# JohnVinyard/music-synthesis

Measured on AMD Instinct MI355X. Metric: GAN train-step audio samples/sec (22.05 kHz, 8192-sample window), higher is better.
Workload: dtype f32 storage and accumulate; multiplies on the 16-bit matrix pipe with split fp32 operands: block-scaled fp16 x 2 (22 significand bits, 3 products per multiply) in the atoms, the k5 layer, the grouped convs, the stride-8 transposed forward and the atom weight gradients; exact bf16 x 3 (6 products) or; 1 GPU; stage-2 GAN train step: alternating D/G trainer calls, MelGAN generator + 3-scale discriminator + feature-matching loss (BASELINE.json configs[2]); per_gpu_batch=32, global_batch=32, window=8192, mels=80, optimizer=FlatAdam(1e-4,(0.5,0.9)), parallelism=dp1, hipgraph=True

## Files before the change

### music-synthesis_amd/csrc/conv5_img.hip

```cpp
#include "operand_split.h"
#include <stdlib.h>

namespace {

constexpr int K5 = 5;
constexpr int PX_MAX = 350;
constexpr int R_MAX = 64;
constexpr int W_NPART = 256;
__host__ __device__ inline size_t c5_tail_u4(int M, int CK) { return (size_t)(M / 32) * (CK / 16) * 5 * 2 * 64; }

__global__ __launch_bounds__(256) void k_conv5_wmax(const float* __restrict__ W, size_t n, float* __restrict__ pm) {
    __shared__ float red[4];
    const size_t per = (n + W_NPART - 1) / W_NPART, lo = blockIdx.x * per, hi = lo + per < n ? lo + per : n;
    float m = 0.f;
    size_t i = lo + 4 * (size_t)threadIdx.x;
    for (; i + 3 < hi; i += 1024) {
        const f32x4u v = *reinterpret_cast<const f32x4u*>(W + i);
        m = fmaxf(fmaxf(m, fmaxf(fabsf(v[0]), fabsf(v[1]))), fmaxf(fabsf(v[2]), fabsf(v[3])));
    }
    for (; i < hi; ++i) m = fmaxf(m, fabsf(W[i]));
#pragma unroll
    for (int o = 32; o > 0; o >>= 1) m = fmaxf(m, __shfl_xor(m, o, 64));
    if ((threadIdx.x & 63) == 0) red[threadIdx.x >> 6] = m;
    __syncthreads();
    if (threadIdx.x == 0) pm[blockIdx.x] = fmaxf(fmaxf(red[0], red[1]), fmaxf(red[2], red[3]));
}

__global__ __launch_bounds__(256) void k_conv5_pack(const float* __restrict__ W, u32x4* __restrict__ img, int M, int CK,
                                                   int backward, int np, const float* __restrict__ pm) {
    const int NC = CK / 16;
    const size_t idx = (size_t)blockIdx.x * 256 + threadIdx.x;
    const size_t total = (size_t)(M / 32) * NC * K5 * 64;
    float WS = 1.f, iWS = 1.f;
    if (np == 2) {
        float* tail = reinterpret_cast<float*>(img + c5_tail_u4(M, CK));
        weight_scale(weight_max256(pm ? pm : tail), WS, iWS);
        if (idx == 0) tail[W_NPART] = iWS;
    }
    if (idx >= total) return;
    const int lane = (int)(idx & 63);
    size_t r = idx >> 6;
    const int tap = (int)(r % K5); r /= K5;
    const int chunk = (int)(r % NC);
    const int ms = (int)(r / NC);
    const int row = ms * 32 + (lane & 31), k0 = chunk * 16 + 8 * (lane >> 5);
    unsigned pc[3][4];
#pragma unroll
    for (int q = 0; q < 4; ++q) {
        float a, b;
        if (!backward) {
            a = W[((size_t)row * CK + k0 + 2 * q) * K5 + tap];
            b = W[((size_t)row * CK + k0 + 2 * q + 1) * K5 + tap];
        } else {
            a = W[((size_t)(k0 + 2 * q) * M + row) * K5 + (K5 - 1 - tap)];
            b = W[((size_t)(k0 + 2 * q + 1) * M + row) * K5 + (K5 - 1 - tap)];
        }
        if (np == 3) {
            unsigned o[3];
            split_pair<3>(a, b, o);
            pc[0][q] = o[0]; pc[1][q] = o[1]; pc[2][q] = o[2];
        } else {
            unsigned o[2];
            split_pair<2>(a * WS, b * WS, o);
            pc[0][q] = o[0]; pc[1][q] = o[1]; pc[2][q] = 0u;
        }
    }
    u32x4* dst = img + ((size_t)((ms * NC + chunk) * K5 + tap) * np) * 64 + lane;
    for (int pp = 0; pp < np; ++pp) dst[pp * 64] = u32x4{pc[pp][0], pc[pp][1], pc[pp][2], pc[pp][3]};
}

struct C5P {
    int B, M, CK, L;
    int R, SS, PX;
    int NV, NVG;
    int cks, nsplit;
    int act;
    float slope;
    long long zstride;
};

extern __shared__ __attribute__((aligned(16))) unsigned char smem5[];

template <int MODE, int NP, bool PRE = false>
__device__ __forceinline__ void conv5_body(const C5P& p, const float* __restrict__ X, const float* __restrict__ Xact,
                                           const u32x4* __restrict__ IMG, const float* __restrict__ bias,
                                           const float* __restrict__ add, float* __restrict__ Y,
                                           float* __restrict__ slabs, int bx, const u32x4* __restrict__ P = nullptr,
                                           const float* __restrict__ Pinv = nullptr) {
    constexpr int XRS = xrs<NP>();
    constexpr bool SC = NP == 2;
    static_assert(!PRE || NP == 2, "pre-split operands are fp16 pieces");
    const int tid = threadIdx.x, lane = tid & 63, h = lane >> 5, l31 = lane & 31;
    const int wid = __builtin_amdgcn_readfirstlane(tid >> 6);
    const int wm = wid >> 2, wn = wid & 3;
    const int L = p.L, b0 = bx * p.R, m0 = blockIdx.y * 64;
    const int cbeg = blockIdx.z * p.cks;
    const int cend = cbeg + p.cks < p.CK ? cbeg + p.cks : p.CK;
    const int nchunks = (cend - cbeg) / 16;
// ... 687 lines not shown
```

### music-synthesis_amd/csrc/conv_thin.hip

```cpp
#include "ms_common.h"
#include "conv_thin.h"
#include <stdlib.h>

namespace {

constexpr int TS = 1024;

template <int K, bool FLIP, bool VEC, int CW>
__global__ __launch_bounds__(256) void k_thin_reduce(int B, int C, int L, int s_kind, int act,
                                                    float slope, const float* __restrict__ S,
                                                    const float* __restrict__ Sact,
                                                    const float* __restrict__ w,
                                                    const float* __restrict__ bias,
                                                    const float* __restrict__ res,
                                                    float* __restrict__ out) {
    constexpr int OFF = (K - 1) / 2;
    constexpr int HV = (OFF + 3) / 4;
    constexpr int NV = 2 * HV + 1;
    constexpr int NW = VEC ? NV * 4 : K + 3;
    constexpr int W0 = VEC ? 4 * HV : OFF;
    __shared__ float red[4][256 + 4];
    const int lane = threadIdx.x & 63, wid = threadIdx.x >> 6;
    const int tiles = (L + 255) / 256;
    const int b = blockIdx.x / tiles, t = (blockIdx.x - b * tiles) * 256 + lane * 4;
// ... 11 lines not shown
                const int tq = t + 4 * (q - HV);
                const bool ok = tq >= 0 && tq < L;
                const float4 v = *reinterpret_cast<const float4*>(S + row + (ok ? tq : 0));
                win[cc][4 * q + 0] = v.x; win[cc][4 * q + 1] = v.y; win[cc][4 * q + 2] = v.z; win[cc][4 * q + 3] = v.w;
            }
        } else {
#pragma unroll
            for (int i = 0; i < K + 3; ++i) {
                const int ti = t + i - OFF;
                const bool ok = ti >= 0 && ti < L;
                win[cc][i] = S[row + (ok ? ti : 0)];
            }
        }
    }
    if (Sact) {
        float wa[CW][NW];
#pragma unroll
        for (int cc = 0; cc < CW; ++cc) {
            const int c = wid * CW + cc;
            const size_t row = ((size_t)b * C + (c < C ? c : 0)) * L;
            if (VEC) {
#pragma unroll
                for (int q = 0; q < NV; ++q) {
                    const int tq = t + 4 * (q - HV);
                    const bool ok = tq >= 0 && tq < L;
                    const float4 v = *reinterpret_cast<const float4*>(Sq + row + (ok ? tq : 0));
                    wa[cc][4 * q + 0] = v.x; wa[cc][4 * q + 1] = v.y; wa[cc][4 * q + 2] = v.z; wa[cc][4 * q + 3] = v.w;
                }
            } else {
#pragma unroll
                for (int i = 0; i < K + 3; ++i) {
                    const int ti = t + i - OFF;
                    const bool ok = ti >= 0 && ti < L;
                    wa[cc][i] = Sq[row + (ok ? ti : 0)];
                }
            }
        }
#pragma unroll
        for (int cc = 0; cc < CW; ++cc)
#pragma unroll
            for (int i = 0; i < NW; ++i) win[cc][i] = ms_act_grad(win[cc][i], wa[cc][i], kind, slope);
    }
#pragma unroll
    for (int cc = 0; cc < CW; ++cc) {
        const int c = wid * CW + cc;
        if (c >= C) continue;
#pragma unroll
        for (int i = 0; i < NW; ++i) {
            const int ti = t + i - W0;
            if (ti < 0 || ti >= L) win[cc][i] = 0.f;
        }
#pragma unroll
        for (int j = 0; j < K; ++j) {
            const float wv = w[c * K + (FLIP ? K - 1 - j : j)];
#pragma unroll
            for (int e = 0; e < 4; ++e) acc[e] = fmaf(wv, win[cc][W0 + e + j - OFF], acc[e]);
        }
    }
#pragma unroll
    for (int e = 0; e < 4; ++e) red[wid][lane * 4 + e] = acc[e];
    __syncthreads();
    const int to = (blockIdx.x - b * tiles) * 256 + threadIdx.x;
    if (to < L) {
        const int i = threadIdx.x;
        float v = (red[0][i] + red[1][i]) + (red[2][i] + red[3][i]);
        v = ms_apply_act(v + (bias ? bias[0] : 0.f), act, slope);
        const size_t o = (size_t)b * L + to;
        if (res) v += res[o];
        out[o] = v;
    }
}

template <int K, bool FLIP, bool VEC, int CW>
__global__ __launch_bounds__(256) void k_thin_expand(int B, int C, int L, int t_kind, int act,
                                                    float slope, const float* __restrict__ T,
                                                    const float* __restrict__ Tact,
                                                    const float* __restrict__ w,
                                                    const float* __restrict__ bias,
                                                    const float* __restrict__ add,
                                                    float* __restrict__ out) {
    constexpr int OFF = (K - 1) / 2;
    const int lane = threadIdx.x & 63, wid = threadIdx.x >> 6;
    const int tiles = (L + 255) / 256;
    const int b = blockIdx.x / tiles, s = (blockIdx.x - b * tiles) * 256 + lane * 4;
    if (s >= L) return;
    const float* Tq = Tact ? Tact : T;
    const int kind = Tact ? t_kind : MS_ACT_NONE;
    float v[K + 3], a[K + 3], win[K + 3];
#pragma unroll
    for (int i = 0; i < K + 3; ++i) {
        const int ti = s + i - OFF;
        const bool ok = ti >= 0 && ti < L;
        v[i] = T[(size_t)b * L + (ok ? ti : 0)];
        a[i] = Tq[(size_t)b * L + (ok ? ti : 0)];
    }
#pragma unroll
    for (int i = 0; i < K + 3; ++i) {
        const int ti = s + i - OFF;
        const bool ok = ti >= 0 && ti < L;
        win[i] = ok ? ms_act_grad(v[i], a[i], kind, slope) : 0.f;
    }
    float4 av[CW];
    if (add && VEC) {
#pragma unroll
        for (int cc = 0; cc < CW; ++cc) {
            const int c = wid * CW + cc;
            av[cc] = *reinterpret_cast<const float4*>(add + ((size_t)b * C + (c < C ? c : 0)) * L + s);
        }
    }
#pragma unroll
    for (int cc = 0; cc < CW; ++cc) {
        const int c = wid * CW + cc;
        if (c >= C) continue;
        float acc[4] = {0.f, 0.f, 0.f, 0.f};
#pragma unroll
        for (int j = 0; j < K; ++j) {
            const float wv = w[c * K + (FLIP ? K - 1 - j : j)];
#pragma unroll
            for (int e = 0; e < 4; ++e) acc[e] = fmaf(wv, win[e + j], acc[e]);
        }
        const float bv = bias ? bias[c] : 0.f;
        const size_t o = ((size_t)b * C + c) * L + s;
        float r[4];
#pragma unroll
        for (int e = 0; e < 4; ++e) r[e] = ms_apply_act(acc[e] + bv, act, slope);
        if (VEC) {
            if (add) { r[0] += av[cc].x; r[1] += av[cc].y; r[2] += av[cc].z; r[3] += av[cc].w; }
            *reinterpret_cast<float4*>(out + o) = make_float4(r[0], r[1], r[2], r[3]);
        } else {
#pragma unroll
            for (int e = 0; e < 4; ++e)
                if (s + e < L) out[o + e] = r[e] + (add ? add[o + e] : 0.f);
        }
    }
}

template <int K, int ROLE, int CPW, bool VEC>
__global__ __launch_bounds__(256) void k_thin_wgrad(int B, int C, int L, int pad, int act, float slope,
                                                   int schunks, const float* __restrict__ S,
                                                   const float* __restrict__ Sact,
                                                   const float* __restrict__ T,
                                                   const float* __restrict__ Tact,
                                                   float* __restrict__ partial, size_t pstride) {
    constexpr int TW = TS + K - 1;
    constexpr int NT = (TW + 255) / 256;
    __shared__ float Tl[NT * 256];
    __shared__ float red[4];
    const int tid = threadIdx.x, lane = tid & 63, wid = tid >> 6;
    const int b = blockIdx.x / schunks, s0 = (blockIdx.x - b * schunks) * TS;
    const int lo = ROLE == 0 ? s0 - (K - 1) + pad : s0 - pad;
    const float* Tq = Tact ? Tact : T;
    const int t_kind = Tact ? act : MS_ACT_NONE;
    const float* Sq = Sact ? Sact : S;
    const int s_kind = Sact ? act : MS_ACT_NONE;
    float bs = 0.f;
    {
        float tv[NT], ta[NT];
#pragma unroll
        for (int it = 0; it < NT; ++it) {
            const int i = tid + it * 256, t = lo + i;
            const bool ok = i < TW && t >= 0 && t < L;
            tv[it] = T[(size_t)b * L + (ok ? t : 0)];
            ta[it] = Tq[(size_t)b * L + (ok ? t : 0)];
        }
#pragma unroll
        for (int it = 0; it < NT; ++it) {
            const int i = tid + it * 256, t = lo + i;
            const bool ok = i < TW && t >= 0 && t < L;
            const float v = ok ? ms_act_grad(tv[it], ta[it], t_kind, slope) : 0.f;
            Tl[i] = v;
            if (ROLE == 0 && ok && t >= s0 && t < s0 + TS) bs += v;
        }
    }
    __syncthreads();
    float acc[CPW][K];
    float bsum[CPW];
#pragma unroll
    for (int cc = 0; cc < CPW; ++cc) {
        bsum[cc] = 0.f;
#pragma unroll
        for (int j = 0; j < K; ++j) acc[cc][j] = 0.f;
    }
    const int c0 = wid * CPW;
#pragma unroll 1
    for (int pass = 0; pass < TS / 256; ++pass) {
        const int sl = pass * 256 + lane * 4, s = s0 + sl;
        float win[K + 3];
#pragma unroll
        for (int i = 0; i < K + 3; ++i) win[i] = Tl[sl + i];
        float4 sv[CPW], sa[CPW];
#pragma unroll
        for (int cc = 0; cc < CPW; ++cc) {
            const int c = c0 + cc;
            const bool ok = c < C && s < L;
            const size_t o = ok ? ((size_t)b * C + c) * L + s : 0;
            if (VEC) {
                sv[cc] = *reinterpret_cast<const float4*>(S + o);
                sa[cc] = *reinterpret_cast<const float4*>(Sq + o);
            } else {
                const size_t o1 = ok && s + 1 < L ? o + 1 : o, o2 = ok && s + 2 < L ? o + 2 : o,
                             o3 = ok && s + 3 < L ? o + 3 : o;
                sv[cc] = make_float4(S[o], S[o1], S[o2], S[o3]);
                sa[cc] = make_float4(Sq[o], Sq[o1], Sq[o2], Sq[o3]);
            }
        }
#pragma unroll
        for (int cc = 0; cc < CPW; ++cc) {
            const int c = c0 + cc;
            const float xv[4] = {sv[cc].x, sv[cc].y, sv[cc].z, sv[cc].w};
            const float xa[4] = {sa[cc].x, sa[cc].y, sa[cc].z, sa[cc].w};
#pragma unroll
            for (int e = 0; e < 4; ++e) {
                const bool ok = c < C && s + e < L;
                const float v = ok ? ms_act_grad(xv[e], xa[e], s_kind, slope) : 0.f;
                bsum[cc] += v;
#pragma unroll
                for (int j = 0; j < K; ++j)
                    acc[cc][j] = fmaf(v, win[ROLE == 0 ? e + K - 1 - j : e + j], acc[cc][j]);
            }
        }
    }
    float* prow = partial + (size_t)blockIdx.x * pstride;
#pragma unroll
    for (int cc = 0; cc < CPW; ++cc) {
        const int c = c0 + cc;
#pragma unroll
        for (int j = 0; j < K; ++j) {
            const float r = ms_wave_sum(acc[cc][j]);
            if (lane == 0 && c < C) prow[c * K + j] = r;
        }
        if (ROLE == 1) {
            const float r = ms_wave_sum(bsum[cc]);
            if (lane == 0 && c < C) prow[(size_t)C * K + c] = r;
        }
    }
    if (ROLE == 0) {
        const float tot = ms_block_sum(bs, red);
        if (tid == 0) prow[(size_t)C * K] = tot;
    }
}

template <int LT>
__global__ __launch_bounds__(256) void k_thin_short_fwd(int C, int L, int act, float slope,
                                                       const float* __restrict__ x,
                                                       const float* __restrict__ w,
                                                       const float* __restrict__ bias,
                                                       float* __restrict__ y) {
    __shared__ float red[4][LT];
    const int tid = threadIdx.x, lane = tid & 63, wid = tid >> 6, b = blockIdx.x;
    float acc[LT];
#pragma unroll
    for (int t = 0; t < LT; ++t) acc[t] = 0.f;
    for (int c = tid; c < C; c += 256) {
        const float w0 = w[c * 3], w1 = w[c * 3 + 1], w2 = w[c * 3 + 2];
        const float* row = x + ((size_t)b * C + c) * L;
        float v[LT + 2];
        v[0] = 0.f;
#pragma unroll
        for (int t = 0; t < LT; ++t) v[t + 1] = t < L ? row[t < L ? t : 0] : 0.f;
        v[LT + 1] = 0.f;
#pragma unroll
        for (int t = 0; t < LT; ++t) acc[t] += w0 * v[t] + w1 * v[t + 1] + w2 * v[t + 2];
    }
#pragma unroll
    for (int t = 0; t < LT; ++t) {
        const float sred = ms_wave_sum(acc[t]);
        if (lane == 0) red[wid][t] = sred;
    }
// ... 331 lines not shown
```

### music-synthesis_amd/csrc/disc_parts.hip

```cpp
#include "operand_split.h"
#include "gconv_mfma.h"
#include <stdint.h>
#include <stdlib.h>

namespace {

constexpr int NP = MS_CONV_PARTS_MAX;

struct DParts {
    int count, wg0[NP + 1];
    int B[NP], L[NP], tiles[NP];
    const float* a[NP];
    const float* b[NP];
    const float* c[NP];
    float* o[NP];
};

struct DPart {
    int B, L, tiles, wg;
    const float* a;
    const float* b;
    const float* c;
    float* o;
};
__device__ __forceinline__ DPart pick_part(const DParts& q, int wg) {
    DPart p{q.B[0], q.L[0], q.tiles[0], wg, q.a[0], q.b[0], q.c[0], q.o[0]};
#pragma unroll
    for (int k = 1; k < NP; ++k)
        if (k < q.count && wg >= q.wg0[k]) p = DPart{q.B[k], q.L[k], q.tiles[k], wg - q.wg0[k], q.a[k], q.b[k], q.c[k], q.o[k]};
    return p;
}

__device__ __forceinline__ float lrelu_grad(float g, float y, float slope) { return y > 0.f ? g : g * slope; }

constexpr int FK = 15, FPAD = 7, FC = 16, FT = 1024;

__device__ __forceinline__ void stage_thin_window(float* xs, const float* x, int B, int L, int b, int tile_t) {
    const auto rs = __builtin_amdgcn_make_buffer_rsrc(const_cast<float*>(x), 0, 4u * (unsigned)(B * L), 0x00020000);
    for (int i = threadIdx.x; i < (FT + 16) / 4; i += 256) {
        const int t = tile_t - 8 + 4 * i;
        *reinterpret_cast<f32x4*>(xs + 4 * i) = load_row4(rs, (unsigned)(b * L), t, L);
    }
    __syncthreads();
}

__global__ __launch_bounds__(256) void k_dfirst_fwd(DParts q, const float* __restrict__ w, const float* __restrict__ bias,
                                                   float slope) {
    __shared__ __attribute__((aligned(16))) float xs[FT + 16];
    const DPart p = pick_part(q, blockIdx.x);
    const int b = p.wg / p.tiles, tile_t = (p.wg - b * p.tiles) * FT;
    stage_thin_window(xs, p.a, p.B, p.L, b, tile_t);
    const int t0 = tile_t + 4 * threadIdx.x;
    if (t0 >= p.L) return;
    float win[20];
#pragma unroll
    for (int i = 0; i < 5; ++i) {
        const f32x4 v = *reinterpret_cast<const f32x4*>(xs + 4 * threadIdx.x + 4 * i);
        win[4 * i] = v[0]; win[4 * i + 1] = v[1]; win[4 * i + 2] = v[2]; win[4 * i + 3] = v[3];
    }
    const bool whole = t0 + 3 < p.L;
#pragma unroll 4
    for (int co = 0; co < FC; ++co) {
        float v[4];
        const float bv = bias ? bias[co] : 0.f;
#pragma unroll
        for (int e = 0; e < 4; ++e) v[e] = bv;
#pragma unroll
        for (int k = 0; k < FK; ++k) {
            const float wk = w[co * FK + k];
#pragma unroll
            for (int e = 0; e < 4; ++e) v[e] = fmaf(wk, win[1 + e + k], v[e]);
        }
#pragma unroll
        for (int e = 0; e < 4; ++e) v[e] = fmaxf(v[e], v[e] * slope);
        float* yr = p.o + ((size_t)b * FC + co) * p.L + t0;
        if (whole) {
            *reinterpret_cast<f32x4u*>(yr) = (f32x4u){v[0], v[1], v[2], v[3]};
        } else {
#pragma unroll
            for (int e = 0; e < 4; ++e)
                if (t0 + e < p.L) yr[e] = v[e];
        }
    }
}

__global__ __launch_bounds__(256) void k_dfirst_bwd_data(DParts q, const float* __restrict__ w, float slope) {
    __shared__ float red[4][256 + 4];
    const DPart p = pick_part(q, blockIdx.x);
    const int lane = threadIdx.x & 63, wid = threadIdx.x >> 6;
    const int b = p.wg / p.tiles, tile_t = (p.wg - b * p.tiles) * 256;
    const int t0 = tile_t + 4 * lane;
    const unsigned bytes = 4u * (unsigned)(p.B * FC * p.L);
    const auto rsG = __builtin_amdgcn_make_buffer_rsrc(const_cast<float*>(p.a), 0, bytes, 0x00020000);
    const auto rsY = __builtin_amdgcn_make_buffer_rsrc(const_cast<float*>(p.b), 0, bytes, 0x00020000);
    float acc[4] = {0.f, 0.f, 0.f, 0.f};
#pragma unroll
    for (int cc = 0; cc < 4; ++cc) {
        const int co = wid * 4 + cc;
        const unsigned row = (unsigned)((b * FC + co) * p.L);
        float win[20];
#pragma unroll
        for (int i = 0; i < 5; ++i) {
            const f32x4 g = load_row4(rsG, row, t0 - 8 + 4 * i, p.L);
            const f32x4 y = load_row4(rsY, row, t0 - 8 + 4 * i, p.L);
#pragma unroll
            for (int e = 0; e < 4; ++e) win[4 * i + e] = lrelu_grad(g[e], y[e], slope);
        }
#pragma unroll
        for (int k = 0; k < FK; ++k) {
            const float wk = w[co * FK + k];
#pragma unroll
            for (int e = 0; e < 4; ++e) acc[e] = fmaf(wk, win[8 + e + FPAD - k], acc[e]);
        }
    }
#pragma unroll
    for (int e = 0; e < 4; ++e) red[wid][4 * lane + e] = acc[e];
    __syncthreads();
    const int to = tile_t + threadIdx.x;
    if (to < p.L) {
        const int i = threadIdx.x;
        float v = (red[0][i] + red[1][i]) + (red[2][i] + red[3][i]);
        if (p.c) v += p.c[(size_t)b * p.L + to];
        p.o[(size_t)b * p.L + to] = v;
    }
}

__global__ __launch_bounds__(256) void k_dfirst_wgrad(DParts q, float slope, float* __restrict__ partial) {
    __shared__ __attribute__((aligned(16))) float xs[FT + 16];
    const int lane = threadIdx.x & 63, wid = threadIdx.x >> 6;
    float acc[4][FK], bsum[4];
#pragma unroll
    for (int cc = 0; cc < 4; ++cc) {
        bsum[cc] = 0.f;
#pragma unroll
        for (int k = 0; k < FK; ++k) acc[cc][k] = 0.f;
    }
    const int nunits = q.wg0[q.count];
    for (int unit = blockIdx.x; unit < nunits; unit += gridDim.x) {
        const DPart p = pick_part(q, unit);
        const int b = p.wg / p.tiles, tile_t = (p.wg - b * p.tiles) * FT;
        __syncthreads();
        stage_thin_window(xs, p.a, p.B, p.L, b, tile_t);
        const unsigned bytes = 4u * (unsigned)(p.B * FC * p.L);
        const auto rsG = __builtin_amdgcn_make_buffer_rsrc(const_cast<float*>(p.b), 0, bytes, 0x00020000);
        const auto rsY = __builtin_amdgcn_make_buffer_rsrc(const_cast<float*>(p.c), 0, bytes, 0x00020000);
#pragma unroll 1
        for (int pass = 0; pass < FT / 256; ++pass) {
            const int sl = pass * 256 + 4 * lane, t0 = tile_t + sl;
            if (tile_t + pass * 256 >= p.L) break;
            float win[20];
#pragma unroll
            for (int i = 0; i < 5; ++i) {
                const f32x4 v = *reinterpret_cast<const f32x4*>(xs + sl + 4 * i);
                win[4 * i] = v[0]; win[4 * i + 1] = v[1]; win[4 * i + 2] = v[2]; win[4 * i + 3] = v[3];
            }
            f32x4 g[4], y[4];
#pragma unroll
            for (int cc = 0; cc < 4; ++cc) {
                const unsigned row = (unsigned)((b * FC + wid * 4 + cc) * p.L);
                g[cc] = load_row4(rsG, row, t0, p.L);
                y[cc] = load_row4(rsY, row, t0, p.L);
            }
#pragma unroll
            for (int cc = 0; cc < 4; ++cc)
#pragma unroll
                for (int e = 0; e < 4; ++e) {
                    const float v = lrelu_grad(g[cc][e], y[cc][e], slope);
                    bsum[cc] += v;
#pragma unroll
                    for (int k = 0; k < FK; ++k) acc[cc][k] = fmaf(v, win[1 + e + k], acc[cc][k]);
                }
        }
    }
    float* prow = partial + (size_t)blockIdx.x * (FC * FK + FC);
#pragma unroll
    for (int cc = 0; cc < 4; ++cc) {
        const int co = wid * 4 + cc;
#pragma unroll
        for (int k = 0; k < FK; ++k) {
            const float r = ms_wave_sum(acc[cc][k]);
            if (lane == 0) prow[co * FK + k] = r;
        }
        const float r = ms_wave_sum(bsum[cc]);
        if (lane == 0) prow[FC * FK + co] = r;
    }
}

__global__ __launch_bounds__(256) void k_dparts_reduce(const float* __restrict__ partial, int nslabs, int stride, int nw,
                                                      int nb, float* __restrict__ gw, float* __restrict__ gb, float beta) {
    const int lane = threadIdx.x & 63, i = blockIdx.x * 4 + (threadIdx.x >> 6);
    if (i >= nw + nb) return;
    float s = 0.f;
    for (int z = lane; z < nslabs; z += 64) s += partial[(size_t)z * stride + i];
    s = ms_wave_sum(s);
    if (lane == 0 && (i < nw || gb)) {
        float* dst = i < nw ? gw + i : gb + (i - nw);
        *dst = (beta != 0.f ? beta * *dst : 0.f) + s;
    }
}

constexpr int JL = 32, JP = 33;

__device__ __forceinline__ void stage_rows(float* lds, const float* __restrict__ src, int L) {
    const int nv = 64 * L;
    const float invL = 1.f / (float)L;
    for (int v = threadIdx.x; v < nv; v += 256) {
        const f32x4 x = *reinterpret_cast<const f32x4*>(src + 4 * v);
        int r = (int)(((float)(4 * v) + 0.5f) * invL);
        int t = 4 * v - r * L;
#pragma unroll
        for (int e = 0; e < 4; ++e) {
            lds[r * JP + t] = x[e];
            if (++t == L) { t = 0; ++r; }
        }
    }
}

__global__ __launch_bounds__(256) void k_djudge_fwd(DParts q, int C, const float* __restrict__ w, const float* __restrict__ bias) {
    __shared__ __attribute__((aligned(16))) float rows[256 * JP];
    __shared__ float red[4][JL];
    const DPart p = pick_part(q, blockIdx.x);
    const int b = p.wg, L = p.L, tid = threadIdx.x, lane = tid & 63, wid = tid >> 6;
    float acc[JL];
#pragma unroll
    for (int t = 0; t < JL; ++t) acc[t] = 0.f;
    for (int c0 = 0; c0 < C; c0 += 256) {
        __syncthreads();
        stage_rows(rows, p.a + ((size_t)b * C + c0) * L, L);
        __syncthreads();
        const float w0 = w[(c0 + tid) * 3], w1 = w[(c0 + tid) * 3 + 1], w2 = w[(c0 + tid) * 3 + 2];
        float v[JL + 2];
        v[0] = 0.f;
#pragma unroll
        for (int t = 0; t < JL; ++t) v[t + 1] = t < L ? rows[tid * JP + t] : 0.f;
        v[JL + 1] = 0.f;
#pragma unroll
        for (int t = 0; t < JL; ++t) acc[t] = fmaf(w2, v[t + 2], fmaf(w1, v[t + 1], fmaf(w0, v[t], acc[t])));
    }
#pragma unroll
    for (int t = 0; t < JL; ++t) {
        const float s = ms_wave_sum(acc[t]);
        if (lane == 0) red[wid][t] = s;
    }
    __syncthreads();
    if (tid < L) p.o[(size_t)b * L + tid] = (red[0][tid] + red[1][tid]) + (red[2][tid] + red[3][tid]) + (bias ? bias[0] : 0.f);
}

__global__ __launch_bounds__(256) void k_djudge_bwd_data(DParts q, int C, const float* __restrict__ w) {
    __shared__ float gj[JL + 2];
    __shared__ float ws[256 * 3];
    const DPart p = pick_part(q, blockIdx.x);
    const int chunks = C / 256, L = p.L, tid = threadIdx.x;
    const int b = p.wg / chunks, c0 = (p.wg - b * chunks) * 256;
    if (tid < JL + 2) {
        const int t = tid - 1;
        gj[tid] = (t >= 0 && t < L) ? p.a[(size_t)b * L + t] : 0.f;
    }
    for (int i = tid; i < 256 * 3; i += 256) ws[i] = w[c0 * 3 + i];
    __syncthreads();
    const size_t base = ((size_t)b * C + c0) * L;
    const float invL = 1.f / (float)L;
    for (int v = tid; v < 64 * L; v += 256) {
        int r = (int)(((float)(4 * v) + 0.5f) * invL);
        int t = 4 * v - r * L;
        f32x4 o;
#pragma unroll
        for (int e = 0; e < 4; ++e) {
            o[e] = fmaf(ws[r * 3], gj[t + 2], fmaf(ws[r * 3 + 1], gj[t + 1], ws[r * 3 + 2] * gj[t]));
            if (++t == L) { t = 0; ++r; }
        }
        if (p.c) o += *reinterpret_cast<const f32x4*>(p.c + base + 4 * v);
        *reinterpret_cast<f32x4*>(p.o + base + 4 * v) = o;
    }
}

__global__ __launch_bounds__(256) void k_djudge_wgrad(DParts q, int C, int nslabs, float* __restrict__ partial) {
    __shared__ __attribute__((aligned(16))) float rows[256 * JP];
    __shared__ float gj[JL + 2];
    __shared__ float red[4];
    const int chunks = C / 256, tid = threadIdx.x;
    const int chunk = blockIdx.x % chunks, slab = blockIdx.x / chunks;
    const int c0 = chunk * 256;
    float a0 = 0.f, a1 = 0.f, a2 = 0.f, bs = 0.f;
    const int nrows = q.wg0[q.count];
    for (int row = slab; row < nrows; row += nslabs) {
        const DPart p = pick_part(q, row);
        const int b = p.wg, L = p.L;
        __syncthreads();
        stage_rows(rows, p.a + ((size_t)b * C + c0) * L, L);
        if (tid < JL + 2) {
            const int t = tid - 1;
            gj[tid] = (t >= 0 && t < L) ? p.b[(size_t)b * L + t] : 0.f;
        }
        __syncthreads();
        for (int t = 0; t < L; ++t) {
            const float x = rows[tid * JP + t];
            a0 = fmaf(x, gj[t + 2], a0);
            a1 = fmaf(x, gj[t + 1], a1);
            a2 = fmaf(x, gj[t], a2);
        }
        if (chunk == 0 && tid < L) bs += gj[tid + 1];
    }
    float* prow = partial + (size_t)slab * (C * 3 + 1);
    prow[(c0 + tid) * 3] = a0; prow[(c0 + tid) * 3 + 1] = a1; prow[(c0 + tid) * 3 + 2] = a2;
    if (chunk == 0) {
        const float tot = ms_block_sum(bs, red);
        if (tid == 0) prow[C * 3] = tot;
    }
}

bool is_first(const ConvP& c) {
    return c.groups == 1 && c.stride == 1 && c.dil == 1 && c.pad_mode == MS_PAD_ZERO && !c.in_act && c.Cin == 1 && c.Cout == FC &&
           c.K == FK && c.pad == FPAD && c.act == MS_ACT_LRELU && c.slope >= 0.f && c.slope <= 1.f;
}
bool is_judge(const ConvP& c) {
    return c.groups == 1 && c.stride == 1 && c.dil == 1 && c.pad_mode == MS_PAD_ZERO && !c.in_act && c.Cout == 1 && c.K == 3 &&
           c.pad == 1 && c.act == MS_ACT_NONE && c.Cin % 256 == 0 && c.Cin >= 256 && c.Cin <= 4096;
}

bool table(const ConvP& c, const ms_conv1d_parts* parts, int tile, int chan, DParts* q) {
    if (!parts || parts->count < 1 || parts->count > NP) return false;
    q->count = parts->count;
    q->wg0[0] = 0;
    for (int i = 0; i < NP; ++i) {
        const bool on = i < parts->count;
        if (on && (parts->B[i] <= 0 || parts->Lin[i] <= 0)) return false;
        if (on && (long long)parts->B[i] * chan * parts->Lin[i] * 4 >= (1ll << 31)) return false;
        q->B[i] = on ? parts->B[i] : 0; q->L[i] = on ? parts->Lin[i] : 1;
        q->tiles[i] = on ? (tile ? ms_ceil_div(parts->Lin[i], tile) : 1) : 1;
        q->wg0[i + 1] = q->wg0[i] + q->B[i] * q->tiles[i];
        q->a[i] = q->b[i] = q->c[i] = nullptr; q->o[i] = nullptr;
    }
    return true;
}

constexpr int FIRST_WGS = 512;
constexpr int JUDGE_SLABS = 48;

}

bool msd_parts_applicable(const ConvP& c, const ms_conv1d_parts* parts, int which) {
    if (!ms_switch_on("MSYNTH_DTHIN")) return false;
    if (!parts || parts->count < 1 || parts->count > NP) return false;
    if (is_first(c)) return true;
    if (!is_judge(c)) return false;
    for (int i = 0; i < parts->count; ++i) {
        if (parts->Lin[i] > JL) return false;
        const uintptr_t a = which == 1 ? (uintptr_t)parts->gx[i] | (uintptr_t)parts->gx_add[i] : (uintptr_t)parts->x[i];
        if (a & 15) return false;
    }
    return true;
}

size_t msd_parts_bwd_weight_ws(const ConvP& c, const ms_conv1d_parts* parts) {
    (void)parts;
    if (is_first(c)) return (size_t)FIRST_WGS * (FC * FK + FC) * sizeof(float);
    return (size_t)JUDGE_SLABS * (c.Cin * 3 + 1) * sizeof(float);
}

int msd_parts_fwd(const ConvP& c, const ms_conv1d_parts* parts, const float* w, const float* bias, hipStream_t s) {
    DParts q;
    const bool first = is_first(c);
    if (!table(c, parts, first ? FT : 0, first ? FC : c.Cin, &q)) return MS_ERR_INVALID_ARG;
    for (int i = 0; i < q.count; ++i) {
        if (!parts->x[i] || !parts->y[i]) return MS_ERR_INVALID_ARG;
        q.a[i] = parts->x[i]; q.o[i] = parts->y[i];
    }
    if (first) {
        ms_note_kernel(0, "k_dfirst_fwd");
        hipLaunchKernelGGL(k_dfirst_fwd, dim3(q.wg0[q.count]), dim3(256), 0, s, q, w, bias, c.slope);
    } else {
        ms_note_kernel(0, "k_djudge_fwd");
        hipLaunchKernelGGL(k_djudge_fwd, dim3(q.wg0[q.count]), dim3(256), 0, s, q, c.Cin, w, bias);
    }
    MS_CHECK_LAUNCH();
    return MS_OK;
}

int msd_parts_bwd_data(const ConvP& c, const ms_conv1d_parts* parts, const float* w, hipStream_t s) {
    DParts q;
    const bool first = is_first(c);
    if (!table(c, parts, first ? 256 : 0, first ? FC : c.Cin, &q)) return MS_ERR_INVALID_ARG;
    for (int i = 0; i < q.count; ++i) {
        if (!parts->gy[i] || !parts->gx[i] || (first && !parts->y_act[i])) return MS_ERR_INVALID_ARG;
        q.a[i] = parts->gy[i]; q.b[i] = parts->y_act[i]; q.c[i] = parts->gx_add[i]; q.o[i] = parts->gx[i];
    }
    if (first) {
        ms_note_kernel(0, "k_dfirst_bwd_data");
        hipLaunchKernelGGL(k_dfirst_bwd_data, dim3(q.wg0[q.count]), dim3(256), 0, s, q, w, c.slope);
    } else {
        const int chunks = c.Cin / 256;
        for (int i = 0; i < NP; ++i) q.wg0[i + 1] = q.wg0[i] + q.B[i] * chunks;
        ms_note_kernel(0, "k_djudge_bwd_data");
        hipLaunchKernelGGL(k_djudge_bwd_data, dim3(q.wg0[q.count]), dim3(256), 0, s, q, c.Cin, w);
    }
    MS_CHECK_LAUNCH();
    return MS_OK;
}

int msd_parts_bwd_weight(const ConvP& c, const ms_conv1d_parts* parts, float* gw, float* gb, float beta, void* ws,
                         size_t ws_bytes, hipStream_t s) {
    DParts q;
    const bool first = is_first(c);
    if (!ws || ws_bytes < msd_parts_bwd_weight_ws(c, parts)) return MS_ERR_WORKSPACE;
    if (!table(c, parts, first ? FT : 0, first ? FC : c.Cin, &q)) return MS_ERR_INVALID_ARG;
    float* partial = (float*)ws;
    if (first) {
        for (int i = 0; i < q.count; ++i) {
            if (!parts->x[i] || !parts->gy[i] || !parts->y_act[i]) return MS_ERR_INVALID_ARG;
            q.a[i] = parts->x[i]; q.b[i] = parts->gy[i]; q.c[i] = parts->y_act[i];
        }
        const int units = q.wg0[q.count];
        const int grid = units < FIRST_WGS ? units : FIRST_WGS;
        ms_note_kernel(0, "k_dfirst_wgrad");
        hipLaunchKernelGGL(k_dfirst_wgrad, dim3(grid), dim3(256), 0, s, q, c.slope, partial);
        MS_CHECK_LAUNCH();
        const int nw = FC * FK, nb = FC;
        hipLaunchKernelGGL(k_dparts_reduce, dim3(ms_ceil_div(nw + nb, 4)), dim3(256), 0, s, partial, grid, nw + nb, nw, nb, gw, gb,
                           beta);
    } else {
        for (int i = 0; i < q.count; ++i) {
            if (!parts->x[i] || !parts->gy[i]) return MS_ERR_INVALID_ARG;
            q.a[i] = parts->x[i]; q.b[i] = parts->gy[i];
        }
        const int rows = q.wg0[q.count], chunks = c.Cin / 256;
        const int slabs = rows < JUDGE_SLABS ? rows : JUDGE_SLABS;
        ms_note_kernel(0, "k_djudge_wgrad");
        hipLaunchKernelGGL(k_djudge_wgrad, dim3(slabs * chunks), dim3(256), 0, s, q, c.Cin, slabs, partial);
        MS_CHECK_LAUNCH();
        const int nw = c.Cin * 3, nb = 1;
        hipLaunchKernelGGL(k_dparts_reduce, dim3(ms_ceil_div(nw + nb, 4)), dim3(256), 0, s, partial, slabs, nw + nb, nw, nb, gw, gb,
                           beta);
    }
    MS_CHECK_LAUNCH();
    return MS_OK;
}
```

### music-synthesis_amd/csrc/elementwise.hip

```cpp
#include "ms_common.h"

namespace {

constexpr int kMaxBlocks = 2048;

inline int grid_for(int64_t n, int per_thread = 4) {
    int64_t b = (n + 256LL * per_thread - 1) / (256LL * per_thread);
    if (b < 1) b = 1;
    if (b > kMaxBlocks) b = kMaxBlocks;
    return (int)b;
}

__global__ __launch_bounds__(256) void k_pool_fwd(const float* __restrict__ x,
                                                 float* __restrict__ y, int64_t rows, int Lin,
                                                 int Lout) {
    const int64_t total = rows * Lout;
    for (int64_t i = (int64_t)blockIdx.x * 256 + threadIdx.x; i < total;
         i += (int64_t)gridDim.x * 256) {
        const int64_t r = i / Lout;
        const int o = (int)(i - r * Lout);
        const float* xr = x + r * Lin;
        const int s = o * 2 - 2;
        float a = 0.f;
#pragma unroll
// ... 372 lines not shown
                                             int64_t n, float lr, float b1, float b2, float eps,
                                             float gscale, const int32_t* __restrict__ step) {
    const double t = (double)step[0];
    const double bc1 = 1.0 - pow((double)b1, t);
    const double bc2 = 1.0 - pow((double)b2, t);
    const float step_size = (float)((double)lr / bc1);
    const float inv_bc2_sqrt = (float)(1.0 / sqrt(bc2));
    const float omb1 = 1.f - b1, omb2 = 1.f - b2;
    const int64_t n4 = n >> 2;
    float4* p4 = reinterpret_cast<float4*>(p);
    const float4* g4 = reinterpret_cast<const float4*>(g);
    float4* m4 = reinterpret_cast<float4*>(m);
    float4* v4 = reinterpret_cast<float4*>(v);
    for (int64_t i = (int64_t)blockIdx.x * 256 + threadIdx.x; i < n4; i += (int64_t)gridDim.x * 256) {
        float4 pp = p4[i], gg = g4[i], mm = m4[i], vv = v4[i];
        float* pa = &pp.x; float* ga = &gg.x; float* ma = &mm.x; float* va = &vv.x;
#pragma unroll
        for (int j = 0; j < 4; ++j) {
            const float gi = ga[j] * gscale;
            ma[j] = b1 * ma[j] + omb1 * gi;
            va[j] = b2 * va[j] + omb2 * gi * gi;
            const float denom = sqrtf(va[j]) * inv_bc2_sqrt + eps;
            pa[j] = pa[j] - step_size * (ma[j] / denom);
        }
        p4[i] = pp; m4[i] = mm; v4[i] = vv;
    }
    for (int64_t i = (n4 << 2) + (int64_t)blockIdx.x * 256 + threadIdx.x; i < n;
         i += (int64_t)gridDim.x * 256) {
        const float gi = g[i] * gscale;
        const float mi = b1 * m[i] + omb1 * gi;
        const float vi = b2 * v[i] + omb2 * gi * gi;
        m[i] = mi; v[i] = vi;
        p[i] = p[i] - step_size * (mi / (sqrtf(vi) * inv_bc2_sqrt + eps));
    }
}

}


namespace {
constexpr int L1M_FWD_EPB = 16384;
struct L1MultiK {
    ms_l1_multi_desc d;
    int blk0[MS_L1_MULTI_MAX + 1];
};

__device__ __forceinline__ int l1m_map(const L1MultiK& k, int blk) {
    int m = 0;
#pragma unroll 1
    for (int i = 1; i < k.d.count; ++i) m = blk >= k.blk0[i] ? i : m;
    return m;
}

__global__ __launch_bounds__(256) void k_l1_multi_fwd(L1MultiK k, float* __restrict__ partials) {
    __shared__ float red[4];
    const int m = l1m_map(k, blockIdx.x);
    const float* r = k.d.r[m];
    const float* f = k.d.f[m];
    const int64_t n = k.d.n[m];
    const int64_t base0 = (int64_t)(blockIdx.x - k.blk0[m]) * L1M_FWD_EPB;
    float s = 0.f;
#pragma unroll 1
    for (int rnd = 0; rnd < L1M_FWD_EPB / 2048; ++rnd) {
        const int64_t base = base0 + (int64_t)rnd * 2048;
        if (base >= n) break;
        float v[8];
#pragma unroll
        for (int i = 0; i < 8; ++i) {
            const int64_t e = base + threadIdx.x + 256 * i;
            const int64_t ec = e < n ? e : 0;
            const float d = f[ec] - r[ec];
            v[i] = e < n ? fabsf(d) : 0.f;
        }
        s += ((v[0] + v[1]) + (v[2] + v[3])) + ((v[4] + v[5]) + (v[6] + v[7]));
    }
    const float tot = ms_block_sum(s, red);
    if (threadIdx.x == 0) partials[blockIdx.x] = tot;
}

__global__ __launch_bounds__(256) void k_l1_multi_final(L1MultiK k, const float* __restrict__ partials,
                                                       float* __restrict__ out) {
    __shared__ float red[4];
    __shared__ float per_map[MS_L1_MULTI_MAX];
    for (int m = threadIdx.x >> 3; m < k.d.count; m += 32) {
        const int sub = threadIdx.x & 7;
        float s = 0.f;
        for (int b = k.blk0[m] + sub; b < k.blk0[m + 1]; b += 8) s += partials[b];
        s += __shfl_xor(s, 1, 64); s += __shfl_xor(s, 2, 64); s += __shfl_xor(s, 4, 64);
        if (sub == 0) per_map[m] = s * k.d.w[m] / (float)k.d.n[m];
    }
    __syncthreads();
    float t = threadIdx.x < k.d.count ? per_map[threadIdx.x] : 0.f;
    const float tot = ms_block_sum(t, red);
    if (threadIdx.x == 0) out[0] = tot;
}

__global__ __launch_bounds__(256) void k_l1_multi_bwd(L1MultiK k, const float* __restrict__ gout,
                                                     float scale) {
    const int m = l1m_map(k, blockIdx.x);
    float* gf = k.d.gf[m];
    if (!gf) return;
    const float* r = k.d.r[m];
    const float* f = k.d.f[m];
    const int64_t n = k.d.n[m];
    const float g = gout[0] * scale * k.d.w[m] / (float)n;
    const int64_t base = (int64_t)(blockIdx.x - k.blk0[m]) * 2048;
    float d[8];
#pragma unroll
    for (int i = 0; i < 8; ++i) {
        const int64_t e = base + threadIdx.x + 256 * i;
        const int64_t ec = e < n ? e : 0;
        d[i] = f[ec] - r[ec];
    }
#pragma unroll
    for (int i = 0; i < 8; ++i) {
        const int64_t e = base + threadIdx.x + 256 * i;
        if (e < n) gf[e] = d[i] > 0.f ? g : (d[i] < 0.f ? -g : 0.f);
    }
}

constexpr int L1M_FB_EPB = 8192;
__global__ __launch_bounds__(256) void k_l1_multi_fwd_bwd(L1MultiK k, float* __restrict__ partials, float gconst) {
    __shared__ float red[4];
    const int m = l1m_map(k, blockIdx.x);
    const float4* r = reinterpret_cast<const float4*>(k.d.r[m]);
    const float4* f = reinterpret_cast<const float4*>(k.d.f[m]);
    float4* gf = reinterpret_cast<float4*>(k.d.gf[m]);
    const int64_t n4 = k.d.n[m] / 4;
    const float g = gconst * k.d.w[m] / (float)k.d.n[m];
    const int64_t base = (int64_t)(blockIdx.x - k.blk0[m]) * (L1M_FB_EPB / 4);
    float4 rv[8], fv[8];
#pragma unroll
    for (int i = 0; i < 8; ++i) {
        const int64_t e = base + threadIdx.x + 256 * i;
        const int64_t ec = e < n4 ? e : 0;
        rv[i] = r[ec]; fv[i] = f[ec];
    }
    float s = 0.f;
#pragma unroll
    for (int i = 0; i < 8; ++i) {
        const int64_t e = base + threadIdx.x + 256 * i;
        const float d0 = fv[i].x - rv[i].x, d1 = fv[i].y - rv[i].y, d2 = fv[i].z - rv[i].z, d3 = fv[i].w - rv[i].w;
        if (e < n4) {
            s += (fabsf(d0) + fabsf(d1)) + (fabsf(d2) + fabsf(d3));
            if (gf) gf[e] = make_float4(d0 > 0.f ? g : (d0 < 0.f ? -g : 0.f), d1 > 0.f ? g : (d1 < 0.f ? -g : 0.f),
                                        d2 > 0.f ? g : (d2 < 0.f ? -g : 0.f), d3 > 0.f ? g : (d3 < 0.f ? -g : 0.f));
        }
    }
    const float tot = ms_block_sum(s, red);
    if (threadIdx.x == 0) partials[blockIdx.x] = tot;
}

bool l1m_plan(const ms_l1_multi_desc* d, L1MultiK* k, int epb = 2048) {
    if (!d || d->count <= 0 || d->count > MS_L1_MULTI_MAX) return false;
    k->d = *d;
    long long blk = 0;
    for (int i = 0; i < d->count; ++i) {
        if (!d->r[i] || !d->f[i] || d->n[i] <= 0) return false;
        k->blk0[i] = (int)blk;
        blk += (d->n[i] + epb - 1) / epb;
        if (blk > (1 << 30)) return false;
    }
    for (int i = d->count; i <= MS_L1_MULTI_MAX; ++i) k->blk0[i] = (int)blk;
    return true;
}
}

extern "C" {

int ms_avg_pool1d_4_2_2_fwd(const float* x, float* y, int64_t rows, int32_t Lin, ms_stream_t stream) {
    if (!x || !y || rows <= 0 || Lin <= 0) return MS_ERR_INVALID_ARG;
    const int Lout = (Lin + 4 - 4) / 2 + 1;
// ... 303 lines not shown
```

Baseline: 109.8 million samples/s.

## Unroll and pipeline loads across several conv and reduction kernels

Several unrelated kernels change. The weight-max reduction is unrolled four times, and the thin-conv expand kernel stages its activation-gradient window in LDS instead of having each lane do redundant global loads. The thin wgrad kernel for K=7 prefetches source rows two passes ahead, and the first discriminator layer's backward-data kernel stages lrelu-gradient windows in shared memory. The judge forward kernel now uses 512 threads with register double-buffering and dynamic LDS, and the L1 final reduction uses whole wavefronts per map. Together these aim to cut redundant memory traffic and expose more load latency hiding, at the cost of more LDS and registers, which may lower occupancy.

Result: no change. 109.3 million samples/s (-0.4%).

```diff
diff --git a/music-synthesis_amd/csrc/conv5_img.hip b/music-synthesis_amd/csrc/conv5_img.hip
--- a/music-synthesis_amd/csrc/conv5_img.hip
+++ b/music-synthesis_amd/csrc/conv5_img.hip
@@ -14,6 +14,14 @@
     const size_t per = (n + W_NPART - 1) / W_NPART, lo = blockIdx.x * per, hi = lo + per < n ? lo + per : n;
     float m = 0.f;
     size_t i = lo + 4 * (size_t)threadIdx.x;
+    for (; i + 3 * 1024 + 3 < hi; i += 4 * 1024) {
+        const f32x4u v0 = *reinterpret_cast<const f32x4u*>(W + i), v1 = *reinterpret_cast<const f32x4u*>(W + i + 1024);
+        const f32x4u v2 = *reinterpret_cast<const f32x4u*>(W + i + 2048), v3 = *reinterpret_cast<const f32x4u*>(W + i + 3072);
+        m = fmaxf(fmaxf(m, fmaxf(fabsf(v0[0]), fabsf(v0[1]))), fmaxf(fabsf(v0[2]), fabsf(v0[3])));
+        m = fmaxf(fmaxf(m, fmaxf(fabsf(v1[0]), fabsf(v1[1]))), fmaxf(fabsf(v1[2]), fabsf(v1[3])));
+        m = fmaxf(fmaxf(m, fmaxf(fabsf(v2[0]), fabsf(v2[1]))), fmaxf(fabsf(v2[2]), fabsf(v2[3])));
+        m = fmaxf(fmaxf(m, fmaxf(fabsf(v3[0]), fabsf(v3[1]))), fmaxf(fabsf(v3[2]), fabsf(v3[3])));
+    }
     for (; i + 3 < hi; i += 1024) {
         const f32x4u v = *reinterpret_cast<const f32x4u*>(W + i);
         m = fmaxf(fmaxf(m, fmaxf(fabsf(v[0]), fabsf(v[1]))), fmaxf(fabsf(v[2]), fabsf(v[3])));
diff --git a/music-synthesis_amd/csrc/conv_thin.hip b/music-synthesis_amd/csrc/conv_thin.hip
--- a/music-synthesis_amd/csrc/conv_thin.hip
+++ b/music-synthesis_amd/csrc/conv_thin.hip
@@ -117,24 +117,31 @@
     constexpr int OFF = (K - 1) / 2;
     const int lane = threadIdx.x & 63, wid = threadIdx.x >> 6;
     const int tiles = (L + 255) / 256;
-    const int b = blockIdx.x / tiles, s = (blockIdx.x - b * tiles) * 256 + lane * 4;
-    if (s >= L) return;
+    const int b = blockIdx.x / tiles, tile = (blockIdx.x - b * tiles) * 256, s = tile + lane * 4;
     const float* Tq = Tact ? Tact : T;
     const int kind = Tact ? t_kind : MS_ACT_NONE;
-    float v[K + 3], a[K + 3], win[K + 3];
-#pragma unroll
-    for (int i = 0; i < K + 3; ++i) {
-        const int ti = s + i - OFF;
-        const bool ok = ti >= 0 && ti < L;
-        v[i] = T[(size_t)b * L + (ok ? ti : 0)];
-        a[i] = Tq[(size_t)b * L + (ok ? ti : 0)];
-    }
-#pragma unroll
-    for (int i = 0; i < K + 3; ++i) {
-        const int ti = s + i - OFF;
-        const bool ok = ti >= 0 && ti < L;
-        win[i] = ok ? ms_act_grad(v[i], a[i], kind, slope) : 0.f;
-    }
+    __shared__ float Ts[2 * 256];
+    {
+        float tv[2], ta[2];
+#pragma unroll
+        for (int it = 0; it < 2; ++it) {
+            const int i = threadIdx.x + 256 * it, ti = tile - OFF + i;
+            const bool ok = i < 256 + K - 1 && ti >= 0 && ti < L;
+            tv[it] = T[(size_t)b * L + (ok ? ti : 0)];
+            ta[it] = Tq[(size_t)b * L + (ok ? ti : 0)];
+        }
+#pragma unroll
+        for (int it = 0; it < 2; ++it) {
+            const int i = threadIdx.x + 256 * it, ti = tile - OFF + i;
+            const bool ok = i < 256 + K - 1 && ti >= 0 && ti < L;
+            if (it == 0 || i < 256 + K - 1) Ts[i] = ok ? ms_act_grad(tv[it], ta[it], kind, slope) : 0.f;
+        }
+    }
+    __syncthreads();
+    if (s >= L) return;
+    float win[K + 3];
+#pragma unroll
+    for (int i = 0; i < K + 3; ++i) win[i] = Ts[lane * 4 + i];
     float4 av[CW];
     if (add && VEC) {
 #pragma unroll
@@ -188,6 +195,18 @@
     const int t_kind = Tact ? act : MS_ACT_NONE;
     const float* Sq = Sact ? Sact : S;
     const int s_kind = Sact ? act : MS_ACT_NONE;
+    const int c0 = wid * CPW;
+    constexpr bool PIPE = VEC && ROLE == 0 && K == 7;
+    auto load_pass = [&](int pass, float4 (&sv)[CPW]) {
+        const int s = s0 + pass * 256 + lane * 4;
+#pragma unroll
+        for (int cc = 0; cc < CPW; ++cc) {
+            const bool ok = c0 + cc < C && s < L;
+            sv[cc] = *reinterpret_cast<const float4*>(S + (ok ? ((size_t)b * C + c0 + cc) * L + s : 0));
+        }
+    };
+    float4 cur[CPW], nx1[CPW];
+    if constexpr (PIPE) { load_pass(0, cur); load_pass(1, nx1); }
     float bs = 0.f;
     {
         float tv[NT], ta[NT];
@@ -216,9 +235,36 @@
 #pragma unroll
         for (int j = 0; j < K; ++j) acc[cc][j] = 0.f;
     }
-    const int c0 = wid * CPW;
+    if constexpr (PIPE) {
+#pragma unroll
+        for (int pass = 0; pass < TS / 256; ++pass) {
+            const int sl = pass * 256 + lane * 4, s = s0 + sl;
+            float4 nx2[CPW];
+            if (pass + 2 < TS / 256) load_pass(pass + 2, nx2);
+            float win[K + 3];
+#pragma unroll
+            for (int i = 0; i < K + 3; ++i) win[i] = Tl[sl + i];
+#pragma unroll
+            for (int cc = 0; cc < CPW; ++cc) {
+                const int c = c0 + cc;
+                const float xv[4] = {cur[cc].x, cur[cc].y, cur[cc].z, cur[cc].w};
+#pragma unroll
+                for (int e = 0; e < 4; ++e) {
+                    const float v = c < C && s + e < L ? xv[e] : 0.f;
+                    bsum[cc] += v;
+#pragma unroll
+                    for (int j = 0; j < K; ++j) acc[cc][j] = fmaf(v, win[e + K - 1 - j], acc[cc][j]);
+                }
+            }
+#pragma unroll
+            for (int cc = 0; cc < CPW; ++cc) {
+                if (pass + 1 < TS / 256) cur[cc] = nx1[cc];
+                if (pass + 2 < TS / 256) nx1[cc] = nx2[cc];
+            }
+        }
+    }
 #pragma unroll 1
-    for (int pass = 0; pass < TS / 256; ++pass) {
+    for (int pass = PIPE ? TS / 256 : 0; pass < TS / 256; ++pass) {
         const int sl = pass * 256 + lane * 4, s = s0 + sl;
         float win[K + 3];
 #pragma unroll
diff --git a/music-synthesis_amd/csrc/disc_parts.hip b/music-synthesis_amd/csrc/disc_parts.hip
--- a/music-synthesis_amd/csrc/disc_parts.hip
+++ b/music-synthesis_amd/csrc/disc_parts.hip
@@ -84,27 +84,48 @@
     }
 }
 
+constexpr int BT = 256, BW = BT + 16;
 __global__ __launch_bounds__(256) void k_dfirst_bwd_data(DParts q, const float* __restrict__ w, float slope) {
     __shared__ float red[4][256 + 4];
+    __shared__ __attribute__((aligned(16))) float gps[4][4][BW];
     const DPart p = pick_part(q, blockIdx.x);
     const int lane = threadIdx.x & 63, wid = threadIdx.x >> 6;
-    const int b = p.wg / p.tiles, tile_t = (p.wg - b * p.tiles) * 256;
-    const int t0 = tile_t + 4 * lane;
+    const int b = p.wg / p.tiles, tile_t = (p.wg - b * p.tiles) * BT;
     const unsigned bytes = 4u * (unsigned)(p.B * FC * p.L);
     const auto rsG = __builtin_amdgcn_make_buffer_rsrc(const_cast<float*>(p.a), 0, bytes, 0x00020000);
     const auto rsY = __builtin_amdgcn_make_buffer_rsrc(const_cast<float*>(p.b), 0, bytes, 0x00020000);
+    {
+        const int ta = tile_t - 8 + 4 * lane;
+        const int tb = lane < 4 ? tile_t - 8 + 256 + 4 * lane : -4;
+        f32x4 ga[4], ya[4], gb[4], yb[4];
+#pragma unroll
+        for (int cc = 0; cc < 4; ++cc) {
+            const unsigned row = (unsigned)((b * FC + wid * 4 + cc) * p.L);
+            ga[cc] = load_row4(rsG, row, ta, p.L); ya[cc] = load_row4(rsY, row, ta, p.L);
+            gb[cc] = load_row4(rsG, row, tb, p.L); yb[cc] = load_row4(rsY, row, tb, p.L);
+        }
+#pragma unroll
+        for (int cc = 0; cc < 4; ++cc) {
+            f32x4 va, vb;
+#pragma unroll
+            for (int e = 0; e < 4; ++e) {
+                va[e] = lrelu_grad(ga[cc][e], ya[cc][e], slope);
+                vb[e] = lrelu_grad(gb[cc][e], yb[cc][e], slope);
+            }
+            *reinterpret_cast<f32x4*>(&gps[wid][cc][4 * lane]) = va;
+            if (lane < 4) *reinterpret_cast<f32x4*>(&gps[wid][cc][256 + 4 * lane]) = vb;
+        }
+    }
+    __syncthreads();
     float acc[4] = {0.f, 0.f, 0.f, 0.f};
 #pragma unroll
     for (int cc = 0; cc < 4; ++cc) {
         const int co = wid * 4 + cc;
-        const unsigned row = (unsigned)((b * FC + co) * p.L);
         float win[20];
 #pragma unroll
         for (int i = 0; i < 5; ++i) {
-            const f32x4 g = load_row4(rsG, row, t0 - 8 + 4 * i, p.L);
-            const f32x4 y = load_row4(rsY, row, t0 - 8 + 4 * i, p.L);
-#pragma unroll
-            for (int e = 0; e < 4; ++e) win[4 * i + e] = lrelu_grad(g[e], y[e], slope);
+            const f32x4 v = *reinterpret_cast<const f32x4*>(&gps[wid][cc][4 * lane + 4 * i]);
+            win[4 * i] = v[0]; win[4 * i + 1] = v[1]; win[4 * i + 2] = v[2]; win[4 * i + 3] = v[3];
         }
 #pragma unroll
         for (int k = 0; k < FK; ++k) {
@@ -216,34 +237,90 @@
     }
 }
 
-__global__ __launch_bounds__(256) void k_djudge_fwd(DParts q, int C, const float* __restrict__ w, const float* __restrict__ bias) {
-    __shared__ __attribute__((aligned(16))) float rows[256 * JP];
-    __shared__ float red[4][JL];
+constexpr int JV = 64 * JL / 256;
+__device__ __forceinline__ void judge_rows_load(f32x4 (&x)[JV], const float* __restrict__ src, int L, int gt) {
+    const int nv = 64 * L;
+#pragma unroll
+    for (int i = 0; i < JV; ++i) {
+        const int v = gt + 256 * i;
+        x[i] = (f32x4){0.f, 0.f, 0.f, 0.f};
+        if (v < nv) x[i] = *reinterpret_cast<const f32x4*>(src + 4 * v);
+    }
+}
+__device__ __forceinline__ void judge_rows_store(float* lds, const f32x4 (&x)[JV], int L, int gt) {
+    const int nv = 64 * L;
+    const float invL = 1.f / (float)L;
+#pragma unroll
+    for (int i = 0; i < JV; ++i) {
+        const int v = gt + 256 * i;
+        if (v < nv) {
+            int r = (int)(((float)(4 * v) + 0.5f) * invL);
+            int t = 4 * v - r * L;
+#pragma unroll
+            for (int e = 0; e < 4; ++e) {
+                lds[r * JP + t] = x[i][e];
+                if (++t == L) { t = 0; ++r; }
+            }
+        }
+    }
+}
+
+constexpr int JG = 2;
+constexpr size_t JFWD_LDS = (size_t)(JG * 256 * JP + JG * 4 * JL) * sizeof(float);
+__global__ __launch_bounds__(JG * 256) void k_djudge_fwd(DParts q, int C, const float* __restrict__ w, const float* __restrict__ bias) {
+    extern __shared__ __attribute__((aligned(16))) float jlds[];
     const DPart p = pick_part(q, blockIdx.x);
-    const int b = p.wg, L = p.L, tid = threadIdx.x, lane = tid & 63, wid = tid >> 6;
+    const int b = p.wg, L = p.L, tid = threadIdx.x, lane = tid & 63, wid = tid >> 6, grp = tid >> 8, gt = tid & 255;
+    float* rows = jlds + grp * 256 * JP;
+    float* red = jlds + JG * 256 * JP;
+    const float* src = p.a + (size_t)b * C * L;
+    constexpr int STEP = JG * 256;
     float acc[JL];
 #pragma unroll
     for (int t = 0; t < JL; ++t) acc[t] = 0.f;
-    for (int c0 = 0; c0 < C; c0 += 256) {
-        __syncthreads();
-        stage_rows(rows, p.a + ((size_t)b * C + c0) * L, L);
-        __syncthreads();
-        const float w0 = w[(c0 + tid) * 3], w1 = w[(c0 + tid) * 3 + 1], w2 = w[(c0 + tid) * 3 + 2];
+    auto consume = [&](int cg) {
+        const float w0 = w[(cg + gt) * 3], w1 = w[(cg + gt) * 3 + 1], w2 = w[(cg + gt) * 3 + 2];
         float v[JL + 2];
         v[0] = 0.f;
 #pragma unroll
-        for (int t = 0; t < JL; ++t) v[t + 1] = t < L ? rows[tid * JP + t] : 0.f;
+        for (int t = 0; t < JL; ++t) v[t + 1] = t < L ? rows[gt * JP + t] : 0.f;
         v[JL + 1] = 0.f;
 #pragma unroll
         for (int t = 0; t < JL; ++t) acc[t] = fmaf(w2, v[t + 2], fmaf(w1, v[t + 1], fmaf(w0, v[t], acc[t])));
+    };
+    f32x4 xa[JV], xb[JV];
+    if (grp * 256 < C) judge_rows_load(xa, src + (size_t)(grp * 256) * L, L, gt);
+    if (grp * 256 + STEP < C) judge_rows_load(xb, src + (size_t)(grp * 256 + STEP) * L, L, gt);
+    for (int c0 = 0; c0 < C; c0 += 2 * STEP) {
+        const int ca = c0 + grp * 256, cb = ca + STEP;
+        if (c0) __syncthreads();
+        if (ca < C) judge_rows_store(rows, xa, L, gt);
+        __syncthreads();
+        if (ca + 2 * STEP < C) judge_rows_load(xa, src + (size_t)(ca + 2 * STEP) * L, L, gt);
+        if (ca < C) consume(ca);
+        if (c0 + STEP < C) {
+            __syncthreads();
+            if (cb < C) judge_rows_store(rows, xb, L, gt);
+            __syncthreads();
+            if (cb + 2 * STEP < C) judge_rows_load(xb, src + (size_t)(cb + 2 * STEP) * L, L, gt);
+            if (cb < C) consume(cb);
+        }
     }
 #pragma unroll
     for (int t = 0; t < JL; ++t) {
         const float s = ms_wave_sum(acc[t]);
-        if (lane == 0) red[wid][t] = s;
+        if (lane == 0) red[wid * JL + t] = s;
     }
     __syncthreads();
-    if (tid < L) p.o[(size_t)b * L + tid] = (red[0][tid] + red[1][tid]) + (red[2][tid] + red[3][tid]) + (bias ? bias[0] : 0.f);
+    if (tid < L) {
+        float s = 0.f;
+#pragma unroll
+        for (int g = 0; g < JG; ++g) {
+            const float* r = red + g * 4 * JL + tid;
+            s += (r[0] + r[JL]) + (r[2 * JL] + r[3 * JL]);
+        }
+        p.o[(size_t)b * L + tid] = s + (bias ? bias[0] : 0.f);
+    }
 }
 
 __global__ __launch_bounds__(256) void k_djudge_bwd_data(DParts q, int C, const float* __restrict__ w) {
@@ -370,8 +447,14 @@
         ms_note_kernel(0, "k_dfirst_fwd");
         hipLaunchKernelGGL(k_dfirst_fwd, dim3(q.wg0[q.count]), dim3(256), 0, s, q, w, bias, c.slope);
     } else {
+        static unsigned long long attr_set = 0;
+        if (ms_first_on_device(attr_set)) {
+            (void)hipFuncSetAttribute(reinterpret_cast<const void*>(&k_djudge_fwd), hipFuncAttributeMaxDynamicSharedMemorySize,
+                                      (int)JFWD_LDS);
+            ms_done_on_device(attr_set);
+        }
         ms_note_kernel(0, "k_djudge_fwd");
-        hipLaunchKernelGGL(k_djudge_fwd, dim3(q.wg0[q.count]), dim3(256), 0, s, q, c.Cin, w, bias);
+        hipLaunchKernelGGL(k_djudge_fwd, dim3(q.wg0[q.count]), dim3(JG * 256), JFWD_LDS, s, q, c.Cin, w, bias);
     }
     MS_CHECK_LAUNCH();
     return MS_OK;
diff --git a/music-synthesis_amd/csrc/elementwise.hip b/music-synthesis_amd/csrc/elementwise.hip
--- a/music-synthesis_amd/csrc/elementwise.hip
+++ b/music-synthesis_amd/csrc/elementwise.hip
@@ -478,12 +478,19 @@
                                                        float* __restrict__ out) {
     __shared__ float red[4];
     __shared__ float per_map[MS_L1_MULTI_MAX];
-    for (int m = threadIdx.x >> 3; m < k.d.count; m += 32) {
-        const int sub = threadIdx.x & 7;
-        float s = 0.f;
-        for (int b = k.blk0[m] + sub; b < k.blk0[m + 1]; b += 8) s += partials[b];
-        s += __shfl_xor(s, 1, 64); s += __shfl_xor(s, 2, 64); s += __shfl_xor(s, 4, 64);
-        if (sub == 0) per_map[m] = s * k.d.w[m] / (float)k.d.n[m];
+    const int lane = threadIdx.x & 63;
+    for (int m = threadIdx.x >> 6; m < k.d.count; m += 4) {
+        const int b0 = k.blk0[m], b1 = k.blk0[m + 1];
+        float s0 = 0.f, s1 = 0.f, s2 = 0.f, s3 = 0.f;
+        for (int b = b0 + lane; b < b1; b += 256) {
+            const float v0 = partials[b];
+            const float v1 = b + 64 < b1 ? partials[b + 64] : 0.f;
+            const float v2 = b + 128 < b1 ? partials[b + 128] : 0.f;
+            const float v3 = b + 192 < b1 ? partials[b + 192] : 0.f;
+            s0 += v0; s1 += v1; s2 += v2; s3 += v3;
+        }
+        const float s = ms_wave_sum((s0 + s1) + (s2 + s3));
+        if (lane == 0) per_map[m] = s * k.d.w[m] / (float)k.d.n[m];
     }
     __syncthreads();
     float t = threadIdx.x < k.d.count ? per_map[threadIdx.x] : 0.f;
```
